# google-deepmind/pycolab

Measured on NVIDIA H100. Metric: env_steps_per_sec, higher is better.
Workload: dtype u8

## Files before the change

### pycolab_b200/csrc/scrolly_maze.cu

```cuda
#include <algorithm>
#include <new>

#include "pcl_device.cuh"
#include "pcl_kernels.cuh"
#include "pcl_crop.cuh"

namespace pcl {

namespace {

constexpr int kS = 4;
constexpr int kWarpsPerBlock = 4;
constexpr int kRecWords = 64;

__device__ __forceinline__ int action_to_motion(int a) {
  constexpr unsigned kTable = (PCL_M_N) | (PCL_M_S << 4) | (PCL_M_W << 8) | (PCL_M_E << 12) |
                              (PCL_M_STAY << 16);
  return (unsigned)a < 5u ? (int)((kTable >> (4 * a)) & 15u) : PCL_M_NONE;
}

__device__ __forceinline__ void cp_async8(void* smem, const void* gmem) {
  asm volatile("cp.async.ca.shared.global [%0], [%1], 8;\n" ::
               "r"((uint32_t)__cvta_generic_to_shared(smem)), "l"(gmem));
}
__device__ __forceinline__ void cp_async16_l1(void* smem, const void* gmem) {
  asm volatile("cp.async.ca.shared.global [%0], [%1], 16;\n" ::
               "r"((uint32_t)__cvta_generic_to_shared(smem)), "l"(gmem));
}


__device__ __forceinline__ int coin_group_shift(int PH) {
  return 32 - __clz((PH - 1) >> 5);
}

__device__ __forceinline__ uint32_t prmt(uint32_t a, uint32_t b, uint32_t sel) {
  uint32_t d;
  asm("prmt.b32 %0, %1, %2, %3;" : "=r"(d) : "r"(a), "r"(b), "r"(sel));
  return d;
}

__host__ __device__ constexpr int window_words(int W) {
  return W < 2 ? 4 : 2 * ((63 + W + 63) / 64);
}

__host__ __device__ constexpr bool narrow_board(int pitch) { return pitch <= 64; }

constexpr int kKeyStride = 16;
enum { kKeyRecWords = 8, kKeyEpoch = 8, kKeySprites = 9, kKeyWords = kKeySprites + kS };
constexpr uint64_t kKeyRec =
    (uint64_t)(48 + PCL_P_FRAME) | (uint64_t)(32 + PCL_D_CORNER_R) << 8 |
    (uint64_t)(32 + PCL_D_CORNER_C) << 16 | (uint64_t)(40 + PCL_D_CORNER_R) << 24 |
    (uint64_t)(40 + PCL_D_CORNER_C) << 32 | (uint64_t)(40 + PCL_D_AUX0) << 40 |
    (uint64_t)(40 + PCL_D_AUX1) << 48 | (uint64_t)(40 + PCL_D_AUX2) << 56;
static_assert(kKeyWords <= kKeyStride, "the render key outgrew its slot");

enum {
  kNbWall = 0,
  kNbCoin = 32,
  kNbBackdrop = 44,
  kNbStart = 56,
  kNbStale = kNbStart + 4 * kS,
  kNbWords = (kNbStale + 2 + 3) & ~3
};

__host__ __device__ constexpr size_t staging_bytes(int H, int W, int pitch) {
  return (size_t)H * pitch + 2 * ((((size_t)H * window_words(W) * 4) + 15) & ~(size_t)15) +
         (narrow_board(pitch) ? 0 : (((size_t)H * (pitch >> 2) + 15) & ~(size_t)15));
}

__host__ __device__ constexpr size_t warp_smem_bytes(int H, int W, int pitch) {
  return kRecWords * 4 + (staging_bytes(H, W, pitch) > (size_t)kNbWords * 4
                             ? staging_bytes(H, W, pitch) : (size_t)kNbWords * 4);
}

__device__ __forceinline__ void pdl_launch_dependents() {
  asm volatile("griddepcontrol.launch_dependents;" ::: "memory");
}
__device__ __forceinline__ void pdl_wait_prior_grids() {
  asm volatile("griddepcontrol.wait;" ::: "memory");
}

struct SelTable { uint16_t v[256]; };
constexpr SelTable make_sel_table() {
  SelTable t = {};
  for (int idx = 0; idx < 256; ++idx) {
    unsigned sel = 0;
    for (int k = 0; k < 4; ++k) {
      const unsigned nib = ((idx >> (4 + k)) & 1) ? 5u : ((idx >> k) & 1) ? 4u : (unsigned)k;
      sel |= nib << (4 * k);
    }
    t.v[idx] = (uint16_t)sel;
  }
  return t;
}
__device__ __align__(16) const SelTable g_sel = make_sel_table();

#ifdef PCL_STEP_STAMPS
constexpr int kStampEnvs = 8192;
enum {
  kStEntry, kStPrior, kStRecords, kStPatch, kStGroup2, kStWait, kStPatched, kStPaint, kStEnd,
  kStTimeIn, kStTimeOut, kStPath, kStampWords
};
enum { kPathDelta, kPathDeltaPickup, kPathFellBack, kPathFull, kPathRestart };
__device__ uint32_t g_stamps[kStampEnvs][kStampWords];
__device__ __forceinline__ uint32_t global_ns() {
  uint32_t t;
  asm volatile("mov.u32 %0, %%globaltimer_lo;" : "=r"(t));
  return t;
}
__device__ __forceinline__ void stamp(int k, uint32_t v) {
  uint32_t tid, cta;
  asm volatile("mov.u32 %0, %%tid.x;" : "=r"(tid));
  asm volatile("mov.u32 %0, %%ctaid.x;" : "=r"(cta));
  const uint32_t e = cta * kWarpsPerBlock + (tid >> 5);
  if ((tid & 31) == 0 && e < (uint32_t)kStampEnvs) g_stamps[e][k] = v;
}
#define PCL_STAMP(k) stamp(k, (uint32_t)clock())
#define PCL_STAMP_TIME(k) stamp(k, global_ns())
#define PCL_STAMP_PATH(v) stamp(kStPath, (uint32_t)(v))
#else
#define PCL_STAMP(k) do {} while (0)
#define PCL_STAMP_TIME(k) do {} while (0)
#define PCL_STAMP_PATH(v) do {} while (0)
#endif

constexpr size_t kMaxBlockSmem = 227 * 1024 - 2048;

static_assert(8 * (kWarpsPerBlock * (warp_smem_bytes(64, 64, 64) + sizeof(SelTable)) + 1024) <=
                  228 * 1024,
              "a 64x64 scrolly_maze block no longer fits 8 times per SM");
static_assert(warp_smem_bytes(1, 1, 16) == kRecWords * 4 + kNbWords * 4,
              "delta rendering's scratch must fit a warp's region on the smallest board");
static_assert(kMaxBlockSmem + kWarpsPerBlock * sizeof(SelTable) == 227 * 1024,
              "kMaxBlockSmem must leave room for the static selector tables");

__device__ __forceinline__ unsigned blocked3x3(int vrow, int vcol, int r0, int c0, unsigned field,
                                               int H, int W, bool p_vis, int p_row, int p_col) {
  const int br = vrow - r0 + 1, bc = vcol - c0 + 1;
  if ((unsigned)br > 2u || (unsigned)bc > 2u) return 0u;
  unsigned colmask = 0;
#pragma unroll
  for (int i = 0; i < 3; ++i) colmask |= ((unsigned)(vcol - 1 + i) < (unsigned)W ? 1u : 0u) << i;
  unsigned blk = 0;
#pragma unroll
  for (int j = 0; j < 3; ++j) {
    unsigned bits = (field >> ((br + j) * 5 + bc)) & colmask;
    if ((unsigned)(vrow - 1 + j) >= (unsigned)H) bits = 0;
    blk |= bits << (3 * j);
  }
  const int dr = p_row - vrow + 1, dc = p_col - vcol + 1;
  if (p_vis && (unsigned)dr <= 2u && (unsigned)dc <= 2u) blk &= ~(1u << (dr * 3 + dc));
  return blk;
}

__device__ __forceinline__ int legal_motions(unsigned b) {
  const unsigned nw = b & 1u, n = (b >> 1) & 1u, ne = (b >> 2) & 1u, w = (b >> 3) & 1u,
                 e = (b >> 5) & 1u, sw = (b >> 6) & 1u, s = (b >> 7) & 1u, se = (b >> 8) & 1u;
  const unsigned blocked = n | ((ne | (n & e)) << 1) | (e << 2) | ((se | (s & e)) << 3) |
                           (s << 4) | ((sw | (s & w)) << 5) | (w << 6) | ((nw | (n & w)) << 7);
  return (int)((~blocked & 0xffu) | (1u << PCL_M_STAY));
}

__device__ __forceinline__ void scrolly_move_p(Drape& d, const ScrollyCfg& cfg, int motion,
                                               Plot& plot, int p_row, int p_col, int p_permit,
                                               int p_permit_frame) {
  if (d.last_frame < plot.frame) {
    d.last_frame = plot.frame;
    d.pre_r = d.corner_r; d.pre_c = d.corner_c;
  }
  const int dr = motion_dr(motion), dc = motion_dc(motion);
  if (plot.order_frame == plot.frame) {
    if (dr != plot.order_r && dc != plot.order_c) plot.error |= PCL_ENV_ERR_ORDER_MISMATCH;
    d.corner_r += plot.order_r; d.corner_c += plot.order_c;
    return;
  }
  if (motion == PCL_M_STAY) return;
  const bool ego = plot.ego_mask & 1;
  const bool possible = !ego || (p_permit_frame == plot.frame && ((p_permit >> motion) & 1));
  int orr, occ;
  if (!cfg.have_margins) {
    if (!possible) return;
    const int nr = d.corner_r + dr, nc = d.corner_c + dc;
    orr = (0 <= nr && nr <= cfg.limit_r) ? dr : 0;
    occ = (0 <= nc && nc <= cfg.limit_c) ? dc : 0;
  } else {
    if (!ego) return;
    const int nr = p_row + dr, nc = p_col + dc;
    const bool want_v = (p_row > nr && nr <= cfg.m_north) || (p_row < nr && nr >= cfg.m_south);
    const bool want_h = (p_col > nc && nc <= cfg.m_west) || (p_col < nc && nc >= cfg.m_east);
    if (!(want_v || want_h)) return;
    orr = want_v ? dr : 0; occ = want_h ? dc : 0;
    const int cr = d.corner_r + orr, cc = d.corner_c + occ;
    if (!((0 <= cr && cr <= cfg.limit_r) && (0 <= cc && cc <= cfg.limit_c)) || !possible) return;
  }
  d.corner_r += orr; d.corner_c += occ;
  plot.order_r = orr; plot.order_c = occ; plot.order_frame = plot.frame;
}

__device__ __forceinline__ int64_t level_of(const StepParams& p, int env) {
  return p.st.d_level ? p.st.d_level[env] : env;
}
__device__ __forceinline__ const uint32_t* level_walls(const StepParams& p, int64_t lvl) {
  return p.st.d_pattern[0] + lvl * p.st.pattern_bstride[0];
}
__device__ __forceinline__ uint32_t* env_coins(const StepParams& p, int env) {
  return p.st.d_pattern[1] + (int64_t)env * p.st.pattern_bstride[1];
}
__device__ __forceinline__ const uint32_t* level_coins(const StepParams& p, int64_t lvl) {
  return p.st.d_pattern_init[1] + lvl * p.st.pattern_init_bstride[1];
}

__device__ __forceinline__ int32_t key_word(const int32_t* rec, int i, uint32_t epoch, int pitch) {
  const int32_t r = rec[i < kKeyRecWords ? (int)((kKeyRec >> (8 * i)) & 0xffu) : 0];
  const int32_t* q = rec + min(max(i - kKeySprites, 0), kS - 1) * PCL_SPRITE_WORDS;
  const int32_t cell = q[PCL_S_FLAGS] & 1 ? q[PCL_S_ROW] * pitch + q[PCL_S_COL] : -1;
  return i < kKeyRecWords ? r : i == kKeyEpoch ? (int32_t)epoch : cell;
}

__global__ void __launch_bounds__(kWarpsPerBlock * 32, 8)
scrolly_maze_step(const StepParams p) {
  extern __shared__ __align__(16) uint8_t smem_raw[];
  PCL_STAMP(kStEntry);
  PCL_STAMP_TIME(kStTimeIn);
  __shared__ __align__(16) uint16_t s_sel_all[kWarpsPerBlock][256];
  const int lane = threadIdx.x & 31;
  const int warp = threadIdx.x >> 5;
  uint16_t* s_sel = s_sel_all[warp];
  pdl_launch_dependents();
  const int env = blockIdx.x * kWarpsPerBlock + warp;
  const bool live = env < p.B;
  const int H = p.H, W = p.W, PWW = p.PWW;
  const int pitch = p.pitch;
  const int nw = window_words(W);

  uint8_t* my = smem_raw + warp * warp_smem_bytes(H, W, pitch);
  int32_t* rec = reinterpret_cast<int32_t*>(my);
  uint8_t* s_bd = my + kRecWords * 4;
  uint32_t* s_wall = reinterpret_cast<uint32_t*>(s_bd + (size_t)H * pitch);
  uint32_t* s_coin = s_wall + ((H * nw + 3) & ~3);
  pdl_wait_prior_grids();
  PCL_STAMP(kStPrior);
  if (p.has_cropper && p.cropper.state && live && lane == 0)
    asm volatile("prefetch.global.L2 [%0];" :: "l"(p.cropper.state + (int64_t)env * 4));
  if (!live) return;
  const int64_t lvl = level_of(p, env);

  int action = env_action(p, env);
  const int32_t key = lane < kKeyWords ? p.render_key[(int64_t)env * kKeyStride + lane] : 0;
  rec[lane] = p.st.d_sprites[(int64_t)env * kS * PCL_SPRITE_WORDS + lane];
  rec[32 + lane] = lane < 16 ? p.st.d_drapes[(int64_t)env * 2 * PCL_DRAPE_WORDS + lane]
                             : p.st.d_plot[(int64_t)env * PCL_PLOT_WORDS + lane - 16];
  __syncwarp();
  PCL_STAMP(kStRecords);
  const int was_over = rec[48 + PCL_P_GAME_OVER];
  bool restart;
  bool frozen = false;
  if (p.mode == MODE_RESET) {
    restart = (p.env_mask == nullptr) || (p.env_mask[env] != 0);
    frozen = !restart;
  } else {
    restart = was_over && p.auto_reset;
    frozen = was_over && !p.auto_reset;
  }
  if (frozen) return;
  const bool key_ok = __all_sync(PCL_FULL, lane >= kKeyWords ||
                                               key == key_word(rec, lane, p.board_epoch, pitch));
  if (restart) {
    const PlotCarry carry = plot_carry(rec + 48, true);
    const unsigned dirty = p.mode == MODE_RESET ? ~0u
                                                : (unsigned)rec[32 + PCL_DRAPE_WORDS + PCL_D_AUX2];
    __syncwarp();
    const int32_t* si = p.st.d_sprites_init + lvl * p.st.sprites_init_bstride;
    const int32_t* di = p.st.d_drapes_init + lvl * p.st.drapes_init_bstride;
    const int32_t* pi = p.st.d_plot_init + lvl * p.st.plot_init_bstride;
    rec[lane] = __ldg(si + lane);
    rec[32 + lane] = lane < 16 ? __ldg(di + lane) : __ldg(pi + lane - 16);
    const uint32_t* src = level_coins(p, lvl);
    const int n = p.PH * PWW, gw = PWW << coin_group_shift(p.PH);
    for (unsigned m = dirty; m != 0u; m &= m - 1u) {
      const int lo = (__ffs(m) - 1) * gw, hi = min(lo + gw, n);
      for (int i = lo + lane; i < hi; i += 32) env_coins(p, env)[i] = __ldg(src + i);
    }
    __syncwarp();
    if (lane == 0) store_carry(rec + 48, carry);
    __syncwarp();
    action = PCL_ACTION_NONE;
  }

  const int me = lane & 3;
  Sprite mine;
  {
    const int32_t* r = rec + me * PCL_SPRITE_WORDS;
    mine.row = r[PCL_S_ROW]; mine.col = r[PCL_S_COL];
    mine.vrow = r[PCL_S_VROW]; mine.vcol = r[PCL_S_VCOL];
    mine.flags = r[PCL_S_FLAGS]; mine.aux0 = r[PCL_S_AUX0]; mine.aux1 = r[PCL_S_AUX1];
    mine.aux2 = 0;
  }
  const int p_row = rec[PCL_S_ROW], p_col = rec[PCL_S_COL];
  const int p_vrow = rec[PCL_S_VROW], p_vcol = rec[PCL_S_VCOL];
  const bool p_vis = rec[PCL_S_FLAGS] & 1;
  const int p_permit = rec[PCL_S_AUX0], p_permit_frame = rec[PCL_S_AUX1];
  const int32_t* rec_coins = rec + 32 + PCL_DRAPE_WORDS;
  Drape walls;
  {
    const int32_t* r = rec + 32;
    walls.corner_r = r[PCL_D_CORNER_R]; walls.corner_c = r[PCL_D_CORNER_C];
    walls.pre_r = r[PCL_D_PRE_R]; walls.pre_c = r[PCL_D_PRE_C];
    walls.last_frame = r[PCL_D_LAST_FRAME];
  }
  Plot plot;
  {
    const int32_t* r = rec + 48;
    plot.frame = r[PCL_P_FRAME]; plot.error = r[PCL_P_ERROR];
    plot.order_r = r[PCL_P_ORDER_R]; plot.order_c = r[PCL_P_ORDER_C];
    plot.order_frame = r[PCL_P_ORDER_FRAME]; plot.ego_mask = r[PCL_P_EGO_MASK];
  }

  const ScrollyCfg wcfg = scrolly_cfg(H, W, p.PH, p.PW, p.margin[0][0], p.margin[0][1]);
  const ScrollyCfg ccfg = scrolly_cfg(H, W, p.PH, p.PW, p.margin[1][0], p.margin[1][1]);
  Directives dir = fresh_directives();
  const int motion = action_to_motion(action);

  plot.frame += 1;

  if (motion != PCL_M_NONE)
    scrolly_move_p(walls, wcfg, motion, plot, p_row, p_col, p_permit, p_permit_frame);
  const bool ordered = plot.order_frame == plot.frame;
  const int wr = walls.corner_r, wc = walls.corner_c;
  const int cr_pred = rec_coins[PCL_D_CORNER_R] + (ordered && motion != PCL_M_NONE ? plot.order_r : 0);
  const int cc_pred = rec_coins[PCL_D_CORNER_C] + (ordered && motion != PCL_M_NONE ? plot.order_c : 0);

  const int we = (wc >> 5) & ~1, ce = (cc_pred >> 5) & ~1;
  const bool narrow = narrow_board(pitch);
  const bool c_touch = rec_coins[PCL_D_LAST_FRAME] < plot.frame;
  const int c_pre_r = rec_coins[c_touch ? PCL_D_CORNER_R : PCL_D_PRE_R];
  const int c_pre_c = rec_coins[c_touch ? PCL_D_CORNER_C : PCL_D_PRE_C];
  unsigned rowbits = 0;
  {
    const uint32_t* row = nullptr;
    int c_first = 0, limit = 0;
    if (lane < 20) {
      const int w = lane / 5, k = lane - w * 5;
      const int pr = wr + rec[w * PCL_SPRITE_WORDS + PCL_S_VROW] + k - 2;
      c_first = wc + rec[w * PCL_SPRITE_WORDS + PCL_S_VCOL] - 2;
      if ((unsigned)pr < (unsigned)p.PH) { row = level_walls(p, lvl) + (int64_t)pr * PWW; limit = PWW; }
    } else if (lane < 24) {
      const int r = lane < 23 ? p_vrow + (lane - 20) - 1 : 0;
      c_first = lane < 23 ? c_pre_c + p_vcol - 1 : c_pre_c;
      if ((unsigned)r < (unsigned)H) {
        const int pr = c_pre_r + r;
        row = ((unsigned)rec_coins[PCL_D_AUX2] >> (pr >> coin_group_shift(p.PH))) & 1u
                  ? env_coins(p, env) : level_coins(p, lvl);
        row += (int64_t)pr * PWW; limit = PWW;
      }
    }
    if (row != nullptr) {
      const int wi = c_first >> 5;
      const uint32_t lo = (unsigned)wi < (unsigned)limit ? row[wi] : 0u;
      const uint32_t hi = (unsigned)(wi + 1) < (unsigned)limit ? row[wi + 1] : 0u;
      rowbits = __funnelshift_r(lo, hi, c_first & 31) & 31u;
    }
  }
  bool delta = key_ok && !restart && wr == rec[32 + PCL_D_CORNER_R] &&
               wc == rec[32 + PCL_D_CORNER_C] && cr_pred == rec_coins[PCL_D_CORNER_R] &&
               cc_pred == rec_coins[PCL_D_CORNER_C] && rec_coins[PCL_D_AUX2] != -1;
  unsigned nb = 0;
  if (delta && lane < 24) {
    const int s = (lane < 12 ? lane : lane - 12) / 3;
    const int vr = rec[s * PCL_SPRITE_WORDS + PCL_S_VROW], vc = rec[s * PCL_SPRITE_WORDS + PCL_S_VCOL];
    const int r = vr + (lane < 12 ? lane : lane - 12) - 3 * s - 1;
    if ((unsigned)r < (unsigned)H) {
      if (lane < 12) {
        const int pr = cr_pred + r, c_first = cc_pred + vc - 1, wi = c_first >> 5;
        const uint32_t* row = ((unsigned)rec_coins[PCL_D_AUX2] >> (pr >> coin_group_shift(p.PH))) & 1u
                                  ? env_coins(p, env) : level_coins(p, lvl);
        row += (int64_t)pr * PWW;
        const uint32_t lo = (unsigned)wi < (unsigned)PWW ? row[wi] : 0u;
        const uint32_t hi = (unsigned)(wi + 1) < (unsigned)PWW ? row[wi + 1] : 0u;
        nb = __funnelshift_r(lo, hi, c_first & 31) & 7u;
      } else {
        const uint8_t* bd = p.st.d_backdrop + lvl * p.st.backdrop_bstride + (int64_t)r * pitch;
#pragma unroll
        for (int j = 0; j < 3; ++j)
          if ((unsigned)(vc - 1 + j) < (unsigned)W) nb |= (unsigned)__ldg(bd + vc - 1 + j) << (8 * j);
      }
    }
  }
  unsigned field = 0;
#pragma unroll
  for (int k = 0; k < 5; ++k) field |= __shfl_sync(PCL_FULL, rowbits, me * 5 + k) << (5 * k);
  unsigned coin9 = 0;
  {
    unsigned colmask = 0;
#pragma unroll
    for (int i = 0; i < 3; ++i)
      colmask |= ((unsigned)(p_vcol - 1 + i) < (unsigned)W ? 1u : 0u) << i;
#pragma unroll
    for (int k = 0; k < 3; ++k) coin9 |= (__shfl_sync(PCL_FULL, rowbits, 20 + k) & colmask) << (3 * k);
    coin9 |= (__shfl_sync(PCL_FULL, rowbits, 23) & 1u) << 9;
  }
  PCL_STAMP(kStPatch);
  uint32_t* s_nb = reinterpret_cast<uint32_t*>(s_bd);
  auto stage = [&](int64_t lvl) {
    cp_async16_l1(reinterpret_cast<uint8_t*>(s_sel) + lane * 16,
                  reinterpret_cast<const uint8_t*>(g_sel.v) + lane * 16);
    {
      const uint8_t* src = p.st.d_backdrop + lvl * p.st.backdrop_bstride + lane * 16;
      uint8_t* dst = s_bd + lane * 16;
      const int n16 = (H * pitch) >> 4;
#pragma unroll 4
      for (int i = lane; i < n16; i += 32, src += 512, dst += 512) cp_async16(dst, src);
    }
    {
      const int gs = coin_group_shift(p.PH);
      const uint32_t* wsrc =
          p.derived[0] + lvl * p.derived_bstride[0] + ((int64_t)(we >> 1) * p.PH + wr) * nw;
      const uint32_t* csrc =
          p.derived[1] + lvl * p.derived_bstride[1] + ((int64_t)(ce >> 1) * p.PH + cr_pred) * nw;
      const int hw = nw >> 1, nhalf = H * hw;
      if (narrow) {
#pragma unroll 1
        for (int r = lane; r < H; r += 32) {
          cp_async16(s_wall + r * 4, wsrc + r * 4);
          if (!(((unsigned)rec_coins[PCL_D_AUX2] >> ((cr_pred + r) >> gs)) & 1u))
            cp_async16(s_coin + r * 4, csrc + r * 4);
        }
      } else {
#pragma unroll 1
        for (int i = lane; i < nhalf; i += 32) {
          const int pr = cr_pred + i / hw;
          cp_async8(s_wall + i * 2, wsrc + i * 2);
          if (!(((unsigned)rec_coins[PCL_D_AUX2] >> (pr >> gs)) & 1u))
            cp_async8(s_coin + i * 2, csrc + i * 2);
        }
      }
      if (rec_coins[PCL_D_AUX2] != 0) {
#pragma unroll 1
        for (int i = lane; i < nhalf; i += 32) {
          const int r = narrow ? i >> 1 : i / hw, k = (i - r * hw) * 2, pr = cr_pred + r;
          if (((unsigned)rec_coins[PCL_D_AUX2] >> (pr >> gs)) & 1u)
            cp_async8(s_coin + i * 2, env_coins(p, env) + (int64_t)pr * PWW + ce + k);
        }
      }
    }
  };
  if (delta) {
    if (lane < 20) s_nb[kNbWall + lane] = rowbits;
    if (lane < 24) s_nb[kNbCoin + lane] = nb;
    if (lane < 4) {
      uint32_t* q = s_nb + kNbStart + 4 * lane;
      q[0] = mine.vrow; q[1] = mine.vcol;
      q[2] = visible(mine) ? mine.row : -1; q[3] = mine.col;
    }
    if (lane < 2) s_nb[kNbStale + lane] = rec_coins[PCL_D_AUX0 + lane];
  } else {
    stage(lvl);
    PCL_STAMP_PATH(restart ? kPathRestart : kPathFull);
  }

  const int r0 = mine.vrow, c0 = mine.vcol;
  const bool is_p = me == 0;
  const bool even = (plot.frame % 2) == 0;
  if (even) scrolly_touch_prescroll(walls, plot);
  int my_err = 0;
  bool hit = false;
  int mot;
  if (is_p) {
    mot = motion;
  } else if (!even) {
    mot = PCL_M_STAY;
  } else {
    const int step = mine.aux0 ? 1 : -1;
    int pr = r0 + walls.pre_r, pc = c0 + walls.pre_c + step;
    bool next_to_wall = false;
    if ((unsigned)pr < (unsigned)p.PH && (unsigned)pc < (unsigned)p.PW) {
      const int dr = pr - wr - r0 + 2, dc = pc - wc - c0 + 2;
      next_to_wall = (field >> (dr * 5 + dc)) & 1u;
    } else {
      if (pr < 0) pr += p.PH;
      if (pc < 0) pc += p.PW;
      if ((unsigned)pr < (unsigned)p.PH && (unsigned)pc < (unsigned)p.PW)
        next_to_wall = bit_at(level_walls(p, level_of(p, env)) + (int64_t)pr * PWW, pc);
      else
        my_err |= PCL_ENV_ERR_INDEX;
    }
    if (next_to_wall) mine.aux0 = !mine.aux0;
    mot = mine.aux0 ? PCL_M_E : PCL_M_W;
  }
  if (mot != PCL_M_NONE) {
    const int dr = motion_dr(mot), dc = motion_dc(mot);
    if (ordered) {
      walker_teleport(mine, H, W, mine.vrow - plot.order_r, mine.vcol - plot.order_c);
      if (is_p && plot.order_r != dr && plot.order_c != dc) my_err |= PCL_ENV_ERR_ORDER_MISMATCH;
    }
    bool legal = true;
    unsigned blk = 0;
    if (mot != PCL_M_STAY || is_p) {
      blk = blocked3x3(mine.vrow, mine.vcol, r0, c0, field, H, W, p_vis, p_row, p_col);
      legal = motion_legal(blk, mot);
    }
    if (legal && mot != PCL_M_STAY) {
      walker_teleport(mine, H, W, mine.vrow + dr, mine.vcol + dc);
      if (is_p) blk = blocked3x3(mine.vrow, mine.vcol, r0, c0, field, H, W, p_vis, p_row, p_col);
    }
    if (is_p) {
      const int valid_at = plot.frame + 1;
      if (mine.aux1 != valid_at) { mine.aux1 = valid_at; mine.aux0 = 0; }
      mine.aux0 |= legal_motions(blk);
    } else if (even) {
      hit = mine.vrow == p_vrow && mine.vcol == p_vcol;
    }
  }
  __syncwarp();
  if (lane < 4) {
    int32_t* r = rec + me * PCL_SPRITE_WORDS;
    r[PCL_S_ROW] = mine.row; r[PCL_S_COL] = mine.col;
    r[PCL_S_VROW] = mine.vrow; r[PCL_S_VCOL] = mine.vcol;
    r[PCL_S_FLAGS] = mine.flags; r[PCL_S_AUX0] = mine.aux0;
    if (is_p) r[PCL_S_AUX1] = mine.aux1;
  }
  if (motion != PCL_M_NONE) plot.ego_mask |= 1;
  plot.error |= __reduce_or_sync(PCL_FULL, (unsigned)(lane < 4 ? my_err : 0));
  if (__any_sync(PCL_FULL, lane < 4 && hit)) terminate(dir);
  Sprite pl;
  pl.row = __shfl_sync(PCL_FULL, mine.row, 0); pl.col = __shfl_sync(PCL_FULL, mine.col, 0);
  pl.vrow = __shfl_sync(PCL_FULL, mine.vrow, 0); pl.vcol = __shfl_sync(PCL_FULL, mine.vcol, 0);
  pl.flags = __shfl_sync(PCL_FULL, mine.flags, 0);
  pl.aux0 = __shfl_sync(PCL_FULL, mine.aux0, 0); pl.aux1 = __shfl_sync(PCL_FULL, mine.aux1, 0);

  Drape coins;
  coins.corner_r = rec_coins[PCL_D_CORNER_R]; coins.corner_c = rec_coins[PCL_D_CORNER_C];
  coins.pre_r = rec_coins[PCL_D_PRE_R]; coins.pre_c = rec_coins[PCL_D_PRE_C];
  coins.last_frame = rec_coins[PCL_D_LAST_FRAME];
  coins.aux0 = rec_coins[PCL_D_AUX0]; coins.aux1 = rec_coins[PCL_D_AUX1];
  scrolly_touch_prescroll(coins, plot);
  plot.aux0 = rec[48 + PCL_P_AUX0];
  int picked_r = -1, picked_c = -1;
  {
    const int dr = pl.row - p_vrow, dc = pl.col - p_vcol;
    bool coin;
    const int pr = coins.pre_r + pl.row, pc = coins.pre_c + pl.col;
    if (pl.row == 0 && pl.col == 0 && !on_board(pl.vrow, pl.vcol, H, W))
      coin = (coin9 >> 9) & 1u;
    else if ((unsigned)(dr + 1) <= 2u && (unsigned)(dc + 1) <= 2u)
      coin = (coin9 >> ((dr + 1) * 3 + dc + 1)) & 1u;
    else
      coin = bit_at(env_coins(p, env) + (int64_t)pr * PWW, pc);
    if (coin) {
      add_reward(dir, 100);
      if (lane == 0) atomicAnd(env_coins(p, env) + (int64_t)pr * PWW + (pc >> 5), ~(1u << (pc & 31)));
      picked_r = pr; picked_c = pc;
      plot.aux0 -= 1;
      if (plot.aux0 == 0) terminate(dir);
      coins.aux0 = pl.row; coins.aux1 = pl.col;
    }
  }
  if (motion != PCL_M_NONE) {
    scrolly_move_p(coins, ccfg, motion, plot, pl.row, pl.col, pl.aux0, pl.aux1);
    coins.aux0 = -1; coins.aux1 = -1;
  } else if (action == 5) {
    terminate(dir);
  }
  PCL_STAMP(kStGroup2);

  cp_async_wait_all();
  PCL_STAMP(kStWait);
  __syncwarp();
  if (lane == 0) {
    int32_t* r = rec + 32;
    r[PCL_D_CORNER_R] = walls.corner_r; r[PCL_D_CORNER_C] = walls.corner_c;
    r[PCL_D_PRE_R] = walls.pre_r; r[PCL_D_PRE_C] = walls.pre_c;
    r[PCL_D_LAST_FRAME] = walls.last_frame;
    r += PCL_DRAPE_WORDS;
    r[PCL_D_CORNER_R] = coins.corner_r; r[PCL_D_CORNER_C] = coins.corner_c;
    r[PCL_D_PRE_R] = coins.pre_r; r[PCL_D_PRE_C] = coins.pre_c;
    r[PCL_D_LAST_FRAME] = coins.last_frame;
    r[PCL_D_AUX0] = coins.aux0; r[PCL_D_AUX1] = coins.aux1;
    r = rec + 48;
    r[PCL_P_FRAME] = plot.frame; r[PCL_P_GAME_OVER] = dir.game_over;
    r[PCL_P_ERROR] = plot.error;
    r[PCL_P_ORDER_R] = plot.order_r; r[PCL_P_ORDER_C] = plot.order_c;
    r[PCL_P_ORDER_FRAME] = plot.order_frame; r[PCL_P_EGO_MASK] = plot.ego_mask;
    r[PCL_P_AUX0] = plot.aux0;
    store_outputs(p.out, env, dir);
    if (picked_r >= 0) rec[32 + PCL_DRAPE_WORDS + PCL_D_AUX2] |= 1 << (picked_r >> coin_group_shift(p.PH));
  }
  const int cr = coins.corner_r, cc = coins.corner_c;

  if (delta) {
    __syncwarp();
    bool fall = cr != cr_pred || cc != cc_pred;
    int cell = -1;
    uint32_t val = 0;
    if (!fall) {
      int r = -1, c = -1;
      if (lane < 4) {
        r = (int)s_nb[kNbStart + 4 * lane + 2]; c = (int)s_nb[kNbStart + 4 * lane + 3];
      } else if (lane < 8) {
        const int32_t* s = rec + (lane - 4) * PCL_SPRITE_WORDS;
        if (s[PCL_S_FLAGS] & 1) { r = s[PCL_S_ROW]; c = s[PCL_S_COL]; }
      } else if (lane == 8) {
        r = (int)s_nb[kNbStale]; c = (int)s_nb[kNbStale + 1];
      } else if (lane == 9) {
        r = rec_coins[PCL_D_AUX0]; c = rec_coins[PCL_D_AUX1];
      } else if (lane == 10 && picked_r >= 0) {
        r = picked_r - cr; c = picked_c - cc;
      }
      bool outside = false;
      if (r >= 0) {
        int s = -1, dr = 0, dc = 0;
#pragma unroll
        for (int t = kS - 1; t >= 0; --t) {
          const int a = r - (int)s_nb[kNbStart + 4 * t] + 1, b = c - (int)s_nb[kNbStart + 4 * t + 1] + 1;
          if ((unsigned)a <= 2u && (unsigned)b <= 2u) { s = t; dr = a; dc = b; }
        }
        outside = s < 0 || !on_board(r, c, H, W);
        if (!outside) {
          const bool wall = (s_nb[kNbWall + 5 * s + dr + 1] >> (dc + 1)) & 1u;
          bool coin = (s_nb[kNbCoin + 3 * s + dr] >> dc) & 1u;
          if (picked_r - cr == r && picked_c - cc == c) coin = false;
          if (rec_coins[PCL_D_AUX0] == r && rec_coins[PCL_D_AUX1] == c) coin = true;
          val = (s_nb[kNbBackdrop + 3 * s + dr] >> (8 * dc)) & 0xffu;
#pragma unroll
          for (int t = 1; t <= kS; ++t) {
            const int32_t* q = rec + (t & 3) * PCL_SPRITE_WORDS;
            if (t == kS && coin) val = '@';
            if (t == kS && wall) val = '#';
            if ((q[PCL_S_FLAGS] & 1) && q[PCL_S_ROW] == r && q[PCL_S_COL] == c) val = p.sprite_char[t & 3];
          }
          cell = r * pitch + c;
        }
      }
      fall = __any_sync(PCL_FULL, outside);
    }
    if (fall) {
      __syncwarp();
      delta = false;
      stage(level_of(p, env));
      cp_async_wait_all();
      PCL_STAMP_PATH(kPathFellBack);
    } else if (cell >= 0) {
      p.out.d_board[(int64_t)env * H * pitch + cell] = (uint8_t)val;
    }
  }

  if (!delta && lane == 0 && picked_r >= 0) {
    const int r2 = picked_r - cr_pred, b = picked_c - (ce << 5);
    if ((unsigned)r2 < (unsigned)H && (unsigned)b < (unsigned)(nw * 32))
      s_coin[r2 * nw + (b >> 5)] &= ~(1u << (b & 31));
  }
  int ce_final = ce;
  if (cr != cr_pred || cc != cc_pred) {
    __syncwarp();
    ce_final = (cc >> 5) & ~1;
    for (int i = lane; i < H * nw; i += 32)
      s_coin[i] = env_coins(p, env)[(int64_t)(cr + i / nw) * PWW + ce_final + i % nw];
  }
  __syncwarp();
  p.st.d_sprites[(int64_t)env * kS * PCL_SPRITE_WORDS + lane] = rec[lane];
  if (lane < 16) p.st.d_drapes[(int64_t)env * 2 * PCL_DRAPE_WORDS + lane] = rec[32 + lane];
  else p.st.d_plot[(int64_t)env * PCL_PLOT_WORDS + lane - 16] = rec[32 + lane];
  if (lane < kKeyWords)
    p.render_key[(int64_t)env * kKeyStride + lane] = key_word(rec, lane, p.board_epoch, pitch);
  if (delta) {
    PCL_STAMP_PATH(picked_r >= 0 ? kPathDeltaPickup : kPathDelta);
    PCL_STAMP(kStPatched);
    PCL_STAMP(kStPaint);
    if (p.has_cropper) {
      __syncwarp();
      crop_epilogue(p.cropper, p.out.d_board, env, lane, rec, rec + 48);
    }
    PCL_STAMP(kStEnd);
    PCL_STAMP_TIME(kStTimeOut);
    return;
  }

  const int spr = pitch >> 4;
  uint32_t* s_seg = narrow ? s_wall : s_coin + ((H * nw + 3) & ~3);
  const int wsh = wc - (we << 5), csh = cc - (ce_final << 5);
  if (narrow) {
    const uint32_t m_lo = W >= 32 ? 0xffffffffu : (1u << W) - 1u;
    const uint32_t m_hi = W >= 64 ? 0xffffffffu : W > 32 ? (1u << (W - 32)) - 1u : 0u;
    for (int r0 = 0; r0 < H; r0 += 32) {
      const int r = min(r0 + lane, H - 1);
      const uint4 wv = *reinterpret_cast<const uint4*>(s_wall + r * 4);
      const uint4 cv = *reinterpret_cast<const uint4*>(s_coin + r * 4);
      const uint32_t wa = (wsh & 32) ? wv.y : wv.x, wb = (wsh & 32) ? wv.z : wv.y,
                     wd = (wsh & 32) ? wv.w : wv.z;
      const uint32_t ca = (csh & 32) ? cv.y : cv.x, cb = (csh & 32) ? cv.z : cv.y,
                     cd = (csh & 32) ? cv.w : cv.z;
      const uint32_t w_lo = __funnelshift_r(wa, wb, wsh & 31) & m_lo;
      const uint32_t w_hi = __funnelshift_r(wb, wd, wsh & 31) & m_hi;
      const uint32_t c_lo = __funnelshift_r(ca, cb, csh & 31) & m_lo;
      const uint32_t c_hi = __funnelshift_r(cb, cd, csh & 31) & m_hi;
      __syncwarp();
      if (r0 + lane < H) {
        uint32_t* out = s_seg + r * spr;
        out[0] = __byte_perm(c_lo, w_lo, 0x5410);
        if (spr > 1) out[1] = __byte_perm(c_lo, w_lo, 0x7632);
        if (spr > 2) out[2] = __byte_perm(c_hi, w_hi, 0x5410);
        if (spr > 3) out[3] = __byte_perm(c_hi, w_hi, 0x7632);
      }
    }
  } else {
    for (int i = lane; i < H * spr; i += 32) {
      const int r = i / spr, j = i - r * spr;
      const int ncols = min(16, W - 16 * j);
      if (ncols <= 0) { s_seg[i] = 0; continue; }
      const uint32_t keep = (1u << ncols) - 1u;
      const int wo = wsh + 16 * j, co = csh + 16 * j;
      const uint32_t* wrow = s_wall + r * nw;
      const uint32_t* crow = s_coin + r * nw;
      const uint32_t w16 = __funnelshift_r(wrow[wo >> 5], (wo >> 5) + 1 < nw ? wrow[(wo >> 5) + 1] : 0u,
                                           wo & 31) & keep;
      const uint32_t c16 = __funnelshift_r(crow[co >> 5], (co >> 5) + 1 < nw ? crow[(co >> 5) + 1] : 0u,
                                           co & 31) & keep;
      s_seg[i] = (w16 << 16) | c16;
    }
  }
  __syncwarp();
  if (lane == 0 && coins.aux0 >= 0)
    s_seg[coins.aux0 * spr + (coins.aux1 >> 4)] |= 1u << (coins.aux1 & 15);
#pragma unroll
  for (int i = 1; i < kS; ++i) {
    if (lane == i && visible(mine)) s_bd[mine.row * pitch + mine.col] = p.sprite_char[i];
    __syncwarp();
  }
  if (lane == 0 && visible(pl)) {
    s_bd[pl.row * pitch + pl.col] = p.sprite_char[0];
    s_seg[pl.row * spr + (pl.col >> 4)] &= ~(0x00010001u << (pl.col & 15));
  }
  __syncwarp();
  PCL_STAMP(kStPatched);
  const int total = H * spr;
  const unsigned drape_chars = ('#' << 8) | '@';
  const uint4* src = reinterpret_cast<const uint4*>(s_bd);
  uint4* dst = reinterpret_cast<uint4*>(p.out.d_board + (int64_t)env * H * pitch);
  for (int seg = lane; seg < total; seg += 32) {
    uint4 px = src[seg];
    const uint32_t bits = s_seg[seg];
    px.x = prmt(px.x, drape_chars, s_sel[((bits >> 12) & 0xf0u) | (bits & 0xfu)]);
    px.y = prmt(px.y, drape_chars, s_sel[((bits >> 16) & 0xf0u) | ((bits >> 4) & 0xfu)]);
    px.z = prmt(px.z, drape_chars, s_sel[((bits >> 20) & 0xf0u) | ((bits >> 8) & 0xfu)]);
    px.w = prmt(px.w, drape_chars, s_sel[((bits >> 24) & 0xf0u) | ((bits >> 12) & 0xfu)]);
    dst[seg] = px;
  }
  PCL_STAMP(kStPaint);
  if (p.has_cropper) {
    __syncwarp();
    crop_epilogue(p.cropper, p.out.d_board, env, lane, rec, rec + 48);
  }
  PCL_STAMP(kStEnd);
  PCL_STAMP_TIME(kStTimeOut);
}

size_t block_smem(int H, int W, int pitch) {
  return warp_smem_bytes(H, W, pitch) * kWarpsPerBlock;
}

int check_spec(const pcl_spec& s) {
  if (!chars_are(s.sprite_char, s.n_sprites, "Pabc")) return PCL_ERR_UNSUPPORTED;
  if (!chars_are(s.drape_char, s.n_drapes, "#@")) return PCL_ERR_UNSUPPORTED;
  if (!chars_are(s.z_order, 6, "abc@#P")) return PCL_ERR_UNSUPPORTED;
  const int lens[3] = {1, 4, 1};
  if (!groups_are(s, "#abcP@", lens, 3)) return PCL_ERR_UNSUPPORTED;
  for (int i = 0; i < 4; ++i) {
    if (!set_is(s.impassable[i], "#")) return PCL_ERR_UNSUPPORTED;
    if (s.sprite_confined[i]) return PCL_ERR_UNSUPPORTED;
    if (s.sprite_egocentric[i] != (i == 0)) return PCL_ERR_UNSUPPORTED;
  }
  if (s.pattern_rows < s.rows || s.pattern_cols < s.cols) return PCL_ERR_INVALID;
  {
    const int nw = window_words(s.cols);
    if ((s.pattern_words & 1) || s.pattern_words < (((s.pattern_cols - s.cols) >> 5) & ~1) + nw ||
        s.pattern_words < (s.pattern_cols + 31) / 32 + 1) return PCL_ERR_INVALID;
    if (block_smem(s.rows, s.cols, s.pitch) > kMaxBlockSmem) return PCL_ERR_UNSUPPORTED;
  }
  for (int d = 0; d < 2; ++d)
    if (!margins_fit(s, d)) return PCL_ERR_INVALID;
  return PCL_OK;
}

int check_state(const pcl_spec&, const pcl_state& st) {
  for (int d = 0; d < 2; ++d) if (!st.d_pattern[d]) return PCL_ERR_INVALID;
  if (!st.d_pattern_init[1] || st.pattern_bstride[1] == 0) return PCL_ERR_INVALID;
  return PCL_OK;
}

CurtainAt curtain(const pcl_spec&, int d) {
  return d == 1 ? CurtainAt::kStaleWindow : CurtainAt::kPatternWindow;
}

cudaError_t launch(const StepParams& p, cudaStream_t s) {
  if (p.PWW & 1) return cudaErrorInvalidValue;
  const size_t smem = block_smem(p.H, p.W, p.pitch);
  if (smem > kMaxBlockSmem) return cudaErrorInvalidValue;
  return launch_step(scrolly_maze_step, p, kWarpsPerBlock, smem, s, true);
}


__global__ void build_blocked(const uint32_t* src, int64_t src_bstride, uint32_t* dst, int PH,
                              int PWW, int nw, int nblk, int64_t total) {
  for (int64_t i = blockIdx.x * (int64_t)blockDim.x + threadIdx.x; i < total;
       i += (int64_t)gridDim.x * blockDim.x) {
    int64_t t = i / nw;
    const int w = (int)(i - t * nw);
    const int row = (int)(t % PH);
    t /= PH;
    const int k = (int)(t % nblk);
    dst[i] = src[(t / nblk) * src_bstride + (int64_t)row * PWW + 2 * k + w];
  }
}

int derive(const pcl_spec& s, const pcl_state& st, int batch, StepParams* p, void** owned) {
  int64_t levels = batch;
  if (st.d_level) {
    int32_t* lv = new (std::nothrow) int32_t[batch];
    if (!lv) return PCL_ERR_NOMEM;
    const cudaError_t e = cudaMemcpy(lv, st.d_level, sizeof(int32_t) * batch, cudaMemcpyDeviceToHost);
    levels = 1;
    for (int i = 0; e == cudaSuccess && i < batch; ++i) levels = std::max<int64_t>(levels, lv[i] + 1);
    delete[] lv;
    if (e != cudaSuccess) return PCL_ERR_CUDA;
  }
  const int W = s.cols, PH = s.pattern_rows;
  const int nw = window_words(W), nblk = ((((s.pattern_cols - W) >> 5) & ~1) >> 1) + 1;
  const int64_t blk_words = (int64_t)nblk * PH * nw;
  const int64_t n_wall = st.pattern_bstride[0] == 0 ? 1 : levels;
  const int64_t n_coin = st.pattern_init_bstride[1] == 0 ? 1 : levels;
  const int64_t off_coin = (n_wall * blk_words * 4 + 255) & ~(int64_t)255;
  const int64_t off_key = (off_coin + n_coin * blk_words * 4 + 255) & ~(int64_t)255;
  uint8_t* buf = nullptr;
  if (cudaMalloc(&buf, off_key + (int64_t)batch * kKeyStride * 4) != cudaSuccess) return PCL_ERR_NOMEM;
  *owned = buf;
  uint32_t* wall = reinterpret_cast<uint32_t*>(buf);
  uint32_t* coin = reinterpret_cast<uint32_t*>(buf + off_coin);
  p->render_key = reinterpret_cast<int32_t*>(buf + off_key);
  if (cudaMemset(p->render_key, 0xff, (size_t)batch * kKeyStride * 4) != cudaSuccess) return PCL_ERR_CUDA;
  build_blocked<<<1024, 256>>>(st.d_pattern[0], st.pattern_bstride[0], wall, PH, s.pattern_words,
                               nw, nblk, n_wall * blk_words);
  build_blocked<<<1024, 256>>>(st.d_pattern_init[1], st.pattern_init_bstride[1], coin, PH,
                               s.pattern_words, nw, nblk, n_coin * blk_words);
  p->derived[0] = wall; p->derived_bstride[0] = n_wall > 1 ? blk_words : 0;
  p->derived[1] = coin; p->derived_bstride[1] = n_coin > 1 ? blk_words : 0;
  return cudaDeviceSynchronize() == cudaSuccess && cudaGetLastError() == cudaSuccess ? PCL_OK
                                                                                     : PCL_ERR_CUDA;
}

}

const Program kScrollyMaze = {check_spec, check_state, curtain, launch, nullptr,
                              false, true,
                              false, nullptr,
                              false, derive};

}

#ifdef PCL_STEP_STAMPS
extern "C" int pcl_step_stamps(uint32_t* host, int n) {
  if (n < 0 || n > pcl::kStampEnvs) return -1;
  return cudaMemcpyFromSymbol(host, pcl::g_stamps, sizeof(pcl::g_stamps[0]) * n) == cudaSuccess
             ? 0 : -3;
}
#endif
```

Measured before the change: 475.6 million.

## Merge wall, coin and backdrop neighbourhood gathers into one lane-parallel load pass

Adds L2 prefetches of per-env sprite, drape, plot and render-key records before the PDL wait, so their latency overlaps the prior grid's tail. It also merges the separate rowbits and delta-path neighbourhood gathers into one pass where every lane issues at most three independent loads. Backdrop bytes are now fetched as aligned words and recombined with a funnel shift across lanes. The delta condition is tightened to require the coin pre-corner to equal the predicted corner, which may route more steps to the full staging path. The new kNbBackdrop slot layout has to match whatever reads it later.

```diff
diff --git a/pycolab_b200/csrc/scrolly_maze.cu b/pycolab_b200/csrc/scrolly_maze.cu
--- a/pycolab_b200/csrc/scrolly_maze.cu
+++ b/pycolab_b200/csrc/scrolly_maze.cu
@@ -238,6 +238,13 @@
   uint8_t* s_bd = my + kRecWords * 4;
   uint32_t* s_wall = reinterpret_cast<uint32_t*>(s_bd + (size_t)H * pitch);
   uint32_t* s_coin = s_wall + ((H * nw + 3) & ~3);
+  if (live && lane < 10) {
+    const int32_t* q = lane < 4 ? p.st.d_sprites + (int64_t)env * kS * PCL_SPRITE_WORDS
+                       : lane < 6 ? p.st.d_drapes + (int64_t)env * 2 * PCL_DRAPE_WORDS
+                       : lane < 8 ? p.st.d_plot + (int64_t)env * PCL_PLOT_WORDS
+                                  : p.render_key + (int64_t)env * kKeyStride;
+    asm volatile("prefetch.global.L2 [%0];" :: "l"(q + 8 * (lane < 4 ? lane : lane & 1)));
+  }
   pdl_wait_prior_grids();
   PCL_STAMP(kStPrior);
   if (p.has_cropper && p.cropper.state && live && lane == 0)
@@ -335,56 +342,48 @@
   const bool c_touch = rec_coins[PCL_D_LAST_FRAME] < plot.frame;
   const int c_pre_r = rec_coins[c_touch ? PCL_D_CORNER_R : PCL_D_PRE_R];
   const int c_pre_c = rec_coins[c_touch ? PCL_D_CORNER_C : PCL_D_PRE_C];
-  unsigned rowbits = 0;
-  {
-    const uint32_t* row = nullptr;
-    int c_first = 0, limit = 0;
-    if (lane < 20) {
-      const int w = lane / 5, k = lane - w * 5;
-      const int pr = wr + rec[w * PCL_SPRITE_WORDS + PCL_S_VROW] + k - 2;
-      c_first = wc + rec[w * PCL_SPRITE_WORDS + PCL_S_VCOL] - 2;
-      if ((unsigned)pr < (unsigned)p.PH) { row = level_walls(p, lvl) + (int64_t)pr * PWW; limit = PWW; }
-    } else if (lane < 24) {
-      const int r = lane < 23 ? p_vrow + (lane - 20) - 1 : 0;
-      c_first = lane < 23 ? c_pre_c + p_vcol - 1 : c_pre_c;
-      if ((unsigned)r < (unsigned)H) {
-        const int pr = c_pre_r + r;
-        row = ((unsigned)rec_coins[PCL_D_AUX2] >> (pr >> coin_group_shift(p.PH))) & 1u
-                  ? env_coins(p, env) : level_coins(p, lvl);
-        row += (int64_t)pr * PWW; limit = PWW;
-      }
-    }
-    if (row != nullptr) {
-      const int wi = c_first >> 5;
-      const uint32_t lo = (unsigned)wi < (unsigned)limit ? row[wi] : 0u;
-      const uint32_t hi = (unsigned)(wi + 1) < (unsigned)limit ? row[wi + 1] : 0u;
-      rowbits = __funnelshift_r(lo, hi, c_first & 31) & 31u;
-    }
-  }
   bool delta = key_ok && !restart && wr == rec[32 + PCL_D_CORNER_R] &&
                wc == rec[32 + PCL_D_CORNER_C] && cr_pred == rec_coins[PCL_D_CORNER_R] &&
-               cc_pred == rec_coins[PCL_D_CORNER_C] && rec_coins[PCL_D_AUX2] != -1;
-  unsigned nb = 0;
-  if (delta && lane < 24) {
-    const int s = (lane < 12 ? lane : lane - 12) / 3;
+               cc_pred == rec_coins[PCL_D_CORNER_C] && rec_coins[PCL_D_AUX2] != -1 &&
+               c_pre_r == cr_pred && c_pre_c == cc_pred;
+  unsigned rowbits;
+  uint32_t c = 0;
+  int bc = 0;
+  {
+    const bool wall = lane < 20;
+    const int s = wall ? lane / 5 : (lane - 20) / 3, k = wall ? lane - 5 * s : lane - 20 - 3 * s;
     const int vr = rec[s * PCL_SPRITE_WORDS + PCL_S_VROW], vc = rec[s * PCL_SPRITE_WORDS + PCL_S_VCOL];
-    const int r = vr + (lane < 12 ? lane : lane - 12) - 3 * s - 1;
-    if ((unsigned)r < (unsigned)H) {
-      if (lane < 12) {
-        const int pr = cr_pred + r, c_first = cc_pred + vc - 1, wi = c_first >> 5;
-        const uint32_t* row = ((unsigned)rec_coins[PCL_D_AUX2] >> (pr >> coin_group_shift(p.PH))) & 1u
-                                  ? env_coins(p, env) : level_coins(p, lvl);
-        row += (int64_t)pr * PWW;
-        const uint32_t lo = (unsigned)wi < (unsigned)PWW ? row[wi] : 0u;
-        const uint32_t hi = (unsigned)(wi + 1) < (unsigned)PWW ? row[wi + 1] : 0u;
-        nb = __funnelshift_r(lo, hi, c_first & 31) & 7u;
-      } else {
-        const uint8_t* bd = p.st.d_backdrop + lvl * p.st.backdrop_bstride + (int64_t)r * pitch;
-#pragma unroll
-        for (int j = 0; j < 3; ++j)
-          if ((unsigned)(vc - 1 + j) < (unsigned)W) nb |= (unsigned)__ldg(bd + vc - 1 + j) << (8 * j);
-      }
-    }
+    const int gs = coin_group_shift(p.PH);
+    const unsigned dirty = (unsigned)rec_coins[PCL_D_AUX2];
+    const int pr = wall ? wr + vr + k - 2 : c_pre_r + vr + k - 1;
+    const int c_first = wall ? wc + vc - 2 : c_pre_c + vc - 1, wi = c_first >> 5;
+    const bool in_row = wall ? (unsigned)pr < (unsigned)p.PH
+                             : (unsigned)(vr + k - 1) < (unsigned)H && (s == 0 || delta);
+    const uint32_t* row = (wall ? level_walls(p, lvl)
+                           : in_row && ((dirty >> (pr >> gs)) & 1u) ? env_coins(p, env)
+                                                                     : level_coins(p, lvl)) +
+                          (int64_t)pr * PWW;
+    const bool qa = in_row && (unsigned)wi < (unsigned)PWW;
+    const bool qb = in_row && (unsigned)(wi + 1) < (unsigned)PWW;
+    const uint32_t* cw =
+        ((dirty >> (c_pre_r >> gs)) & 1u ? env_coins(p, env) : level_coins(p, lvl)) +
+        (int64_t)c_pre_r * PWW + (c_pre_c >> 5);
+    bool qc = lane == 24 && (unsigned)(c_pre_c >> 5) < (unsigned)PWW;
+    if (delta && lane < 24) {
+      const int j = lane < 12 ? lane : lane - 12, bs = j / 3;
+      const int br = rec[bs * PCL_SPRITE_WORDS + PCL_S_VROW] + j - 3 * bs - 1;
+      bc = rec[bs * PCL_SPRITE_WORDS + PCL_S_VCOL] - 1;
+      const int bw = (bc >> 2) + (lane < 12 ? 0 : 1);
+      cw = reinterpret_cast<const uint32_t*>(p.st.d_backdrop + lvl * p.st.backdrop_bstride +
+                                             (int64_t)br * pitch) + bw;
+      qc = (unsigned)br < (unsigned)H && (unsigned)bw < (unsigned)(pitch >> 2) &&
+           (lane < 12 || (bc & 3) > 1);
+    }
+    uint32_t a = 0, b = 0;
+    if (qa) a = row[wi];
+    if (qb) b = row[wi + 1];
+    if (qc) c = *cw;
+    rowbits = __funnelshift_r(a, b, c_first & 31) & 31u;
   }
   unsigned field = 0;
 #pragma unroll
@@ -397,7 +396,7 @@
       colmask |= ((unsigned)(p_vcol - 1 + i) < (unsigned)W ? 1u : 0u) << i;
 #pragma unroll
     for (int k = 0; k < 3; ++k) coin9 |= (__shfl_sync(PCL_FULL, rowbits, 20 + k) & colmask) << (3 * k);
-    coin9 |= (__shfl_sync(PCL_FULL, rowbits, 23) & 1u) << 9;
+    coin9 |= ((__shfl_sync(PCL_FULL, c, 24) >> (c_pre_c & 31)) & 1u) << 9;
   }
   PCL_STAMP(kStPatch);
   uint32_t* s_nb = reinterpret_cast<uint32_t*>(s_bd);
@@ -446,7 +445,12 @@
   };
   if (delta) {
     if (lane < 20) s_nb[kNbWall + lane] = rowbits;
-    if (lane < 24) s_nb[kNbCoin + lane] = nb;
+    else s_nb[kNbCoin + lane - 20] = rowbits & 7u;
+    const uint32_t c_next = __shfl_down_sync(PCL_FULL, c, 12);
+    unsigned keep = 0;
+#pragma unroll
+    for (int i = 0; i < 3; ++i) keep |= ((unsigned)(bc + i) < (unsigned)W ? 0xffu : 0u) << (8 * i);
+    if (lane < 12) s_nb[kNbBackdrop + lane] = __funnelshift_r(c, c_next, 8 * (bc & 3)) & keep;
     if (lane < 4) {
       uint32_t* q = s_nb + kNbStart + 4 * lane;
       q[0] = mine.vrow; q[1] = mine.vcol;
```

Result: no change. 480.3 million (median of 6 runs) (+1.0%).

## Merge per-lane bit-row gathers into two branchless predicated loads

Applied to the files above, without the earlier changes.

Replaces the two divergent per-lane gather phases (wall/coin rowbits, then delta neighbour coins and byte-wise backdrop) with two uniform predicated-load phases. Pointer selection uses selp and loads are guarded by predicates, and the second word is skipped when the bit window fits in one word. Coin neighbour bits are reused from the first phase by requiring the pre-scroll corner to equal the predicted corner for the delta path. Backdrop bytes are fetched as a 32-bit funnel-shifted word. The goal is to cut warp divergence and serial dependent loads, at the cost of a stricter delta condition that may send more steps to the full staging path. It also changes the shared-memory slot layout (kNbBackdrop).

```diff
diff --git a/pycolab_b200/csrc/scrolly_maze.cu b/pycolab_b200/csrc/scrolly_maze.cu
--- a/pycolab_b200/csrc/scrolly_maze.cu
+++ b/pycolab_b200/csrc/scrolly_maze.cu
@@ -28,6 +28,27 @@
                "r"((uint32_t)__cvta_generic_to_shared(smem)), "l"(gmem));
 }
 
+
+__device__ __forceinline__ uint32_t ld_global_if(bool c, const uint32_t* a) {
+  uint32_t v;
+  asm("{ .reg .pred q; .reg .u64 g; setp.ne.b32 q, %2, 0; cvta.to.global.u64 g, %1;\n\t"
+      "mov.u32 %0, 0; @q ld.global.u32 %0, [g]; }"
+      : "=r"(v) : "l"(a), "r"((int)c));
+  return v;
+}
+__device__ __forceinline__ void bits_load(const uint32_t* row, int bit, int n, int width,
+                                          uint32_t& lo, uint32_t& hi) {
+  const int wi = bit >> 5;
+  lo = ld_global_if((unsigned)wi < (unsigned)n, row + wi);
+  hi = ld_global_if((unsigned)(wi + 1) < (unsigned)n && (bit & 31) + width > 32, row + wi + 1);
+}
+
+__device__ __forceinline__ const uint32_t* select_ptr(bool c, const uint32_t* a, const uint32_t* b) {
+  const uint32_t* d;
+  asm("{ .reg .pred q; setp.ne.b32 q, %3, 0; selp.b64 %0, %1, %2, q; }"
+      : "=l"(d) : "l"(a), "l"(b), "r"((int)c));
+  return d;
+}
 
 __device__ __forceinline__ int coin_group_shift(int PH) {
   return 32 - __clz((PH - 1) >> 5);
@@ -335,56 +356,50 @@
   const bool c_touch = rec_coins[PCL_D_LAST_FRAME] < plot.frame;
   const int c_pre_r = rec_coins[c_touch ? PCL_D_CORNER_R : PCL_D_PRE_R];
   const int c_pre_c = rec_coins[c_touch ? PCL_D_CORNER_C : PCL_D_PRE_C];
-  unsigned rowbits = 0;
-  {
-    const uint32_t* row = nullptr;
-    int c_first = 0, limit = 0;
-    if (lane < 20) {
-      const int w = lane / 5, k = lane - w * 5;
-      const int pr = wr + rec[w * PCL_SPRITE_WORDS + PCL_S_VROW] + k - 2;
-      c_first = wc + rec[w * PCL_SPRITE_WORDS + PCL_S_VCOL] - 2;
-      if ((unsigned)pr < (unsigned)p.PH) { row = level_walls(p, lvl) + (int64_t)pr * PWW; limit = PWW; }
-    } else if (lane < 24) {
-      const int r = lane < 23 ? p_vrow + (lane - 20) - 1 : 0;
-      c_first = lane < 23 ? c_pre_c + p_vcol - 1 : c_pre_c;
-      if ((unsigned)r < (unsigned)H) {
-        const int pr = c_pre_r + r;
-        row = ((unsigned)rec_coins[PCL_D_AUX2] >> (pr >> coin_group_shift(p.PH))) & 1u
-                  ? env_coins(p, env) : level_coins(p, lvl);
-        row += (int64_t)pr * PWW; limit = PWW;
-      }
-    }
-    if (row != nullptr) {
-      const int wi = c_first >> 5;
-      const uint32_t lo = (unsigned)wi < (unsigned)limit ? row[wi] : 0u;
-      const uint32_t hi = (unsigned)(wi + 1) < (unsigned)limit ? row[wi + 1] : 0u;
-      rowbits = __funnelshift_r(lo, hi, c_first & 31) & 31u;
-    }
-  }
   bool delta = key_ok && !restart && wr == rec[32 + PCL_D_CORNER_R] &&
                wc == rec[32 + PCL_D_CORNER_C] && cr_pred == rec_coins[PCL_D_CORNER_R] &&
-               cc_pred == rec_coins[PCL_D_CORNER_C] && rec_coins[PCL_D_AUX2] != -1;
-  unsigned nb = 0;
-  if (delta && lane < 24) {
-    const int s = (lane < 12 ? lane : lane - 12) / 3;
+               cc_pred == rec_coins[PCL_D_CORNER_C] && rec_coins[PCL_D_AUX2] != -1 &&
+               c_pre_r == cr_pred && c_pre_c == cc_pred;
+  uint32_t lo_a, hi_a, lo_b, hi_b;
+  int bit_a, bit_b;
+  {
+    const bool wall = lane < 20;
+    const int s = wall ? lane / 5 : (lane - 20) / 3, k = wall ? lane - 5 * s : lane - 20 - 3 * s;
     const int vr = rec[s * PCL_SPRITE_WORDS + PCL_S_VROW], vc = rec[s * PCL_SPRITE_WORDS + PCL_S_VCOL];
-    const int r = vr + (lane < 12 ? lane : lane - 12) - 3 * s - 1;
-    if ((unsigned)r < (unsigned)H) {
-      if (lane < 12) {
-        const int pr = cr_pred + r, c_first = cc_pred + vc - 1, wi = c_first >> 5;
-        const uint32_t* row = ((unsigned)rec_coins[PCL_D_AUX2] >> (pr >> coin_group_shift(p.PH))) & 1u
-                                  ? env_coins(p, env) : level_coins(p, lvl);
-        row += (int64_t)pr * PWW;
-        const uint32_t lo = (unsigned)wi < (unsigned)PWW ? row[wi] : 0u;
-        const uint32_t hi = (unsigned)(wi + 1) < (unsigned)PWW ? row[wi + 1] : 0u;
-        nb = __funnelshift_r(lo, hi, c_first & 31) & 7u;
-      } else {
-        const uint8_t* bd = p.st.d_backdrop + lvl * p.st.backdrop_bstride + (int64_t)r * pitch;
+    const int r = vr + k - (wall ? 2 : 1);
+    int pr = wall ? wr + r : c_pre_r + r;
+    const bool ok = wall ? (unsigned)pr < (unsigned)p.PH
+                         : (unsigned)r < (unsigned)H && (s == 0 || delta);
+    pr = ok ? pr : 0;
+    bit_a = (wall ? wc - 1 : c_pre_c) + vc - 1;
+    const bool env_row = ((unsigned)rec_coins[PCL_D_AUX2] >> (pr >> coin_group_shift(p.PH))) & 1u;
+    const uint32_t* row =
+        select_ptr(wall, level_walls(p, lvl), select_ptr(env_row, env_coins(p, env), level_coins(p, lvl))) +
+        (int64_t)pr * PWW;
+    bits_load(row, bit_a, ok ? PWW : 0, wall ? 5 : 3, lo_a, hi_a);
+  }
+  {
+    const bool bd = lane < 12;
+    const int s = min(lane / 3, kS - 1), k = lane - 3 * s;
+    const int vr = rec[s * PCL_SPRITE_WORDS + PCL_S_VROW], vc = rec[s * PCL_SPRITE_WORDS + PCL_S_VCOL];
+    const int r = vr + k - 1;
+    const bool ok = bd ? delta && (unsigned)r < (unsigned)H && (unsigned)(vc + 1) <= (unsigned)W + 1u
+                       : lane == 12;
+    bit_b = bd ? (ok ? 8 * (r * pitch + vc - 1) : 0) : c_pre_c;
+    const bool env_row = ((unsigned)rec_coins[PCL_D_AUX2] >> (c_pre_r >> coin_group_shift(p.PH))) & 1u;
+    const uint32_t* row = select_ptr(
+        bd, reinterpret_cast<const uint32_t*>(p.st.d_backdrop + lvl * p.st.backdrop_bstride),
+        select_ptr(env_row, env_coins(p, env), level_coins(p, lvl)) + (int64_t)c_pre_r * PWW);
+    bits_load(row, bit_b, ok ? (bd ? (H * pitch) >> 2 : PWW) : 0, bd ? 24 : 1, lo_b, hi_b);
+  }
+  const unsigned rowbits = __funnelshift_r(lo_a, hi_a, bit_a & 31) & 31u;
+  unsigned nb = __funnelshift_r(lo_b, hi_b, bit_b & 31);
+  if (lane < 12) {
+    const int vc = rec[(lane / 3) * PCL_SPRITE_WORDS + PCL_S_VCOL];
+    unsigned keep = 0;
 #pragma unroll
-        for (int j = 0; j < 3; ++j)
-          if ((unsigned)(vc - 1 + j) < (unsigned)W) nb |= (unsigned)__ldg(bd + vc - 1 + j) << (8 * j);
-      }
-    }
+    for (int j = 0; j < 3; ++j) keep |= ((unsigned)(vc - 1 + j) < (unsigned)W ? 0xffu : 0u) << (8 * j);
+    nb &= keep;
   }
   unsigned field = 0;
 #pragma unroll
@@ -397,7 +412,7 @@
       colmask |= ((unsigned)(p_vcol - 1 + i) < (unsigned)W ? 1u : 0u) << i;
 #pragma unroll
     for (int k = 0; k < 3; ++k) coin9 |= (__shfl_sync(PCL_FULL, rowbits, 20 + k) & colmask) << (3 * k);
-    coin9 |= (__shfl_sync(PCL_FULL, rowbits, 23) & 1u) << 9;
+    coin9 |= (__shfl_sync(PCL_FULL, nb, 12) & 1u) << 9;
   }
   PCL_STAMP(kStPatch);
   uint32_t* s_nb = reinterpret_cast<uint32_t*>(s_bd);
@@ -446,7 +461,8 @@
   };
   if (delta) {
     if (lane < 20) s_nb[kNbWall + lane] = rowbits;
-    if (lane < 24) s_nb[kNbCoin + lane] = nb;
+    else s_nb[kNbCoin + lane - 20] = rowbits & 7u;
+    if (lane < 12) s_nb[kNbBackdrop + lane] = nb;
     if (lane < 4) {
       uint32_t* q = s_nb + kNbStart + 4 * lane;
       q[0] = mine.vrow; q[1] = mine.vcol;
```

New measurement: 470.7 million before, 471.9 million after (median of 6 runs). Within noise of the previous version (+0.3%).
